# s-will/BiAlign

Hardware: AMD Instinct MI355X
Metric: giga-DP-cells/sec (higher is better)
Workload: dtype int32

## Files before the change

### bialign_amd/csrc/bialign_capi.hip

```cpp
#include "bialign_host.hpp"
#include <cmath>
#include <cstdint>
#include <unordered_map>

using namespace bialign;

namespace bialign {

static thread_local std::string g_err;

int fail(int code, const char* fmt, ...) {
  char buf[512];
  va_list ap;
  va_start(ap, fmt);
  vsnprintf(buf, sizeof buf, fmt, ap);
  va_end(ap);
  g_err = buf;
  return code;
}

struct SweepInfo {
  int W, R, RR, MAXOFF, PADB;
  int recdw, lean_recdw;
  int blk, min_goff;
// ... 434 lines not shown
  for (int t = 0; t < sc->k1 * sc->k1; ++t) amax = std::max<int64_t>(amax, std::llabs((long long)sc->s1[t]));
  int64_t bmax = 0;
  for (int t = 0; t < sc->k2 * sc->k2; ++t) bmax = std::max<int64_t>(bmax, std::llabs((long long)sc->s2[t]));
  auto dense_max = [&](const int32_t* tab, const int64_t* off) {
    int64_t mx = 0;
    for (int p = 0; p < pr->npairs; ++p) {
      const int64_t cnt = (int64_t)std::max(pr->len_a[p], 0) * std::max(pr->len_b[p], 0);
      for (int64_t t = 0; t < cnt; ++t) mx = std::max<int64_t>(mx, std::llabs((long long)tab[off[p] + t]));
    }
    return mx;
  };
  if (b->dense && !b->feat) bmax = dense_max(pr->mu2_dense, pr->mu2_off);
  if (b->feat) {
    struct MolMax { int32_t len; double up, down, unp; };
    std::unordered_map<int64_t, MolMax> seen[2];
    auto check = [&](int side, int p, int64_t off, int32_t len, const double* up, const double* down, const double* unp,
                     const MolMax** res) {
      MolMax& mm = seen[side][off];
      if (mm.len < len) {
        const double* arr[3] = {up, down, unp};
        static const char* const names[3] = {"up", "down", "unp"};
        double mx[3] = {0, 0, 0};
        for (int f = 0; f < 3; ++f)
          for (int32_t r = 0; r < len; ++r) {
            const double x = arr[f][off + r];
            if (!(x >= 0.0) || std::isinf(x))
              return fail(BIALIGN_E_INVALID, "pair %d: feature %s_%c at position %d is %g: features must be finite and >= 0", p,
                          names[f], side ? 'b' : 'a', r + 1, x);
            mx[f] = std::max(mx[f], x);
          }
        mm = MolMax{len, mx[0], mx[1], mx[2]};
      }
      *res = &mm;
      return BIALIGN_OK;
    };
    bmax = 0;
    for (int p = 0; p < pr->npairs; ++p) {
      const MolMax *ma = nullptr, *mb = nullptr;
      if (int rc = check(0, p, pr->off_a[p], std::max(pr->len_a[p], 0), ft->up_a, ft->down_a, ft->unp_a, &ma)) return rc;
      if (int rc = check(1, p, pr->off_b[p], std::max(pr->len_b[p], 0), ft->up_b, ft->down_b, ft->unp_b, &mb)) return rc;
      const double bound = std::fabs((double)ft->structure_weight) *
                           (std::sqrt(ma->up * mb->up) + std::sqrt(ma->down * mb->down) + std::sqrt(ma->unp * mb->unp));
      if (!(bound < 1073741824.0))
        return fail(BIALIGN_E_RANGE, "pair %d: structure scores may leave the int32 safety window (bound %g)", p, bound);
      bmax = std::max<int64_t>(bmax, (int64_t)std::ceil(bound));
    }
  }
  if (b->dense1) amax = dense_max(pr->mu1_dense, pr->mu1_off);
  const int64_t colmax = amax + bmax + 2 * (std::llabs((long long)prm->gap_cost) + std::llabs((long long)prm->gap_opening_cost)) +
                         2 * std::llabs((long long)prm->shift_cost);

  int64_t tot_a = 0, tot_b = 0, tot_tab = 0;
  b->pairs.resize(pr->npairs);
  std::vector<int64_t> pair_dwords(pr->npairs);
  for (int p = 0; p < pr->npairs; ++p) {
    const int n = pr->len_a[p], m = pr->len_b[p];
    if (n < 1 || m < 1)
      return fail(BIALIGN_E_INVALID, "pair %d: empty molecule (n=%d, m=%d)", p, n, m);
    if ((2 * ((int64_t)n + m) + 8) * colmax >= (1 << 28))
      return fail(BIALIGN_E_RANGE, "pair %d: scores may leave the int32 safety window (n+m=%d, column bound %lld)", p,
                  n + m, (long long)colmax);
    PairDesc& d = b->pairs[p];
    d.n = n;
    d.m = m;
    d.NS = d.P = d.G = 0;
    if (!b->wide) sweep_geometry(geo, n, m, &d.NS, &d.P, &d.G);
    d.trace_cap = 2 * (n + m) + 2;
    d.seq_a = pr->off_a[p];
    d.seq_b = pr->off_b[p];
    d.trace_off = b->trace_bytes;
    d.tab_off = tot_tab;
    tot_tab += (int64_t)n * m * ((b->dense ? 1 : 0) + (b->dense1 ? 1 : 0));
    if (b->feat) b->tab_dwords.push_back((int64_t)n * m * (b->dense1 ? 2 : 1));
    b->trace_bytes += d.trace_cap;
    b->cells += cells_of(n, m, S);
    tot_a = std::max<int64_t>(tot_a, pr->off_a[p] + n);
    tot_b = std::max<int64_t>(tot_b, pr->off_b[p] + m);
    if (!b->wide) {
      b->lds_bytes = std::max(b->lds_bytes, lds_need(geo, 1, sc->k1, sc->k2, n, m, b->dense, false, b->dense1));
      b->lds_base = std::max(b->lds_base, lds_need(geo, 0, sc->k1, sc->k2, n, m, b->dense, false, b->dense1));
      b->lds_diet8 = std::max(b->lds_diet8, lds_need(geo, 8, sc->k1, sc->k2, n, m, false, true));
      b->lds_slim_codes = std::max(b->lds_slim_codes, lds_need_slim_codes(geo, n, m));
    }
    b->lds_trace = std::max<size_t>(b->lds_trace, ((size_t)sc->k1 * sc->k1 + (size_t)sc->k2 * sc->k2) * 4 +
                                                      (b->dense1 ? 1 : 2) * ((size_t)code_pad(n) + (size_t)code_pad(m)));
  }
  if (!b->wide)
    b->lds_per_wave = lds_need(geo, 1, sc->k1, sc->k2, 1, 1, b->dense, false, b->dense1) -
                      lds_need(geo, 0, sc->k1, sc->k2, 1, 1, b->dense, false, b->dense1);
  if (!b->wide) b->lds_slim_base = lds_need_slim_base(geo, sc->k1, sc->k2);
  if (std::max(b->lds_bytes, b->lds_trace) > 160 * 1024)
    return fail(BIALIGN_E_UNSUPPORTED, "molecules too long for the LDS staging (%zu bytes needed, 160 KiB per workgroup)",
                std::max(b->lds_bytes, b->lds_trace));

  {
    const char* e = getenv("BIALIGN_PACK");
    const bool force = e && e[0] == '1';
    const PackInfo pki = pack_info(S);
    bool ok = b->affine && S >= 1 && S <= BIALIGN_MAX_SHIFT_PACKED && !b->lean && !b->dense1 && prm->gap_opening_cost <= 0 &&
              !(e && e[0] == '0') &&
              (force || colmax < 8192) &&
              (force || S < 3 || pr->npairs >= 64);
    for (int p = 0; ok && p < pr->npairs; ++p) {
      const PairDesc& d = b->pairs[p];
      const int interior = d.m - S - pki.lo + 1;
      const int64_t packed_dw = pki.written_dwords(d.G, d.P, d.m);
      const int64_t full_dw = (int64_t)d.G * pki.full_recdw;
      ok = interior >= 1 && (force || packed_dw * 5 <= full_dw * 4);
    }
    b->pack = ok;
  }

  size_t free_b = 0, total_b = 0;
  HIP_TRY(hipMemGetInfo(&free_b, &total_b));
  free_b += (eng->layer_cache.n + eng->layer_cache2.n) * sizeof(int32_t);
  if (b->feat) free_b += eng->tab_cache.n * sizeof(int32_t);
  int64_t budget = hbm_budget > 0 ? hbm_budget : (int64_t)(free_b * 0.85);
  budget = std::min<int64_t>(budget, (int64_t)(free_b * 0.95));
  const int64_t budget_dw = budget / 4;
  auto size_pairs = [&]() {
    for (int p = 0; p < pr->npairs; ++p) {
      PairDesc& d = b->pairs[p];
      if (b->wide) {
        pair_dwords[p] = b->lean ? 16 : wide_pair_dwords(d.n, d.m, S, b->NL);
        continue;
      }
      const int64_t lean_dw = (int64_t)d.G * geo.lean_recdw;
      const int64_t scratch_dw = (int64_t)(d.m + geo.MAXOFF + 1) * geo.recdw;
      d.scratch_off = lean_dw;
      pair_dwords[p] = b->lean_trace ? lean_dw + b->resw_k * scratch_dw : (b->lean ? lean_dw : (int64_t)d.G * geo.recdw);
      if (b->pack && !b->lean)
        pair_dwords[p] = pack_info(S).pair_dwords(d.G, d.P, d.m);
    }
  };
  auto max_need = [&]() {
    int64_t mx = 0;
    for (int p = 0; p < pr->npairs; ++p) mx = std::max(mx, pair_dwords[p] + (b->feat ? b->tab_dwords[p] : 0));
    return mx;
  };
  auto pick_resw_k = [&]() {
    int ns_max = 1;
    for (const PairDesc& d : b->pairs) ns_max = std::max(ns_max, d.NS);
    b->resw_k = (int)std::min<int64_t>(std::min<int64_t>(256, std::max(1, ns_max / 4)), std::max<int64_t>(1, 2048 / pr->npairs));
    if (const char* e = getenv("BIALIGN_RESW_K")) b->resw_k = std::min(256, std::max(1, atoi(e)));
    for (size_pairs(); b->resw_k > 1 && max_need() > budget_dw; size_pairs())
      b->resw_k /= 2;
  };
  if (b->lean_trace) pick_resw_k();
  size_pairs();
  if (b->pack) {
    int64_t full_max = 0;
    for (int p = 0; p < pr->npairs; ++p)
      full_max = std::max(full_max, (int64_t)b->pairs[p].G * pack_info(S).full_recdw + (b->feat ? b->tab_dwords[p] : 0));
    if (std::max(full_max, max_need()) > budget_dw) {
      b->pack = false;
      size_pairs();
    }
  }
  if (!b->lean && !b->wide && max_need() > budget_dw) {
    b->lean = b->lean_trace = true;
    b->pack = false;
    pick_resw_k();
  }
  b->full_dwords.resize(pr->npairs);
  for (int p = 0; p < pr->npairs; ++p) b->full_dwords[p] = b->wide ? pair_dwords[p] : (int64_t)b->pairs[p].G * geo.recdw;
  b->packed_sizing = b->pack && !b->lean;
  if (int rc = plan_chunks(b.get(), pair_dwords, budget_dw)) return rc;

// ... 438 lines not shown
```

### bialign_amd/csrc/bialign_host.hpp

```cpp
#pragma once
#include "bialign_kernels.hpp"

#include <algorithm>
#include <cstdarg>
#include <cstdio>
#include <cstdlib>
#include <cstring>
#include <memory>
#include <mutex>
#include <numeric>
#include <string>
#include <type_traits>
#include <vector>

#include "../../include/bialign.h"

#define BIALIGN_MAX_SHIFT_PACKED 3

namespace bialign {

int fail(int code, const char* fmt, ...);

#define HIP_TRY(expr)                                                                 \
  do {                                                                                \
// ... 313 lines not shown
  constexpr int PPW = 12 / TW;
  DeviceBatch w = v;
  w.order = v.order + first;
  w.team = 1;
  w.launch_pairs = count;
  w.slim_code_bytes = (int32_t)b->lds_slim_codes;
  b->packed_layers = !LEAN;
  if (!LEAN) b->used_pack = true;
  b->last_team = TW;
  return launch(fill_affine_slim_kernel<S, TW, PPW, LEAN>, dim3((count + PPW - 1) / PPW), dim3(64 * 12), b->lds_slim(TW),
                b->eng->stream, w);
}

template <int S, bool LEAN>
int launch_fill_affine_slim(bialign_batch* b, const DeviceBatch& v, int first, int count, int tw) {
  switch (tw) {
    case 2: return launch_fill_affine_slim_t<S, 2, LEAN>(b, v, first, count);
    case 3: return launch_fill_affine_slim_t<S, 3, LEAN>(b, v, first, count);
    case 6: return launch_fill_affine_slim_t<S, 6, LEAN>(b, v, first, count);
    case 12: return launch_fill_affine_slim_t<S, 12, LEAN>(b, v, first, count);
  }
  return fail(BIALIGN_E_UNSUPPORTED, "no three-waves-per-SIMD sweep for max_shift %d, team %d", S, tw);
}

template <int S, int TW, unsigned F>
int xcu_resident_affine(bialign_batch* b) {
  constexpr unsigned Q = (F & ~F_PACK) | F_XCU;
  if constexpr (fill_affine_exists(S, TW, Q)) {
    if (TW == 8 && !diet8_available(b)) return 0;
    return xcu_resident_cached(b, ((F & F_LEAN) ? 1 : 0) + (TW == 8 ? 2 : 0), fill_affine_of<S, TW, Q>(), 64 * TW, fill_lds<S, TW>(b, true));
  } else {
    return 0;
  }
}

template <int S, int TW, unsigned F>
bool fill_affine_rung(bialign_batch* b, const DeviceBatch& v, int first, int count, const TeamShape& ts, int* rc) {
  if constexpr (fill_affine_exists(S, TW, F)) {
    constexpr bool XCU = (F & F_XCU) != 0;
    if (XCU ? !(ts.gw > 1 && (TW == 1 || ts.tw == TW)) : ts.tw < TW) return false;
    *rc = launch_fill_affine_t<S, TW, F>(b, v, first, count, XCU ? ts.gw : 1);
    return true;
  } else {
    return false;
  }
}

template <int S>
int launch_fill_affine(bialign_batch* b, const DeviceBatch& v, int first, int count) {
  return with_flags<F_DENSE | F_LEAN | F_PACK | F_DENSE1 | F_BETA_ANY>(fill_flags(b), [&](auto flags) -> int {
    constexpr unsigned F = decltype(flags)::value;
    if constexpr (!fill_affine_exists(S, 1, F)) {
      return fail(BIALIGN_E_UNSUPPORTED, "no affine sweep for max_shift %d in form %u", S, F);
    } else {
      TeamShape ts;
      if constexpr (!(F & F_BETA_ANY)) ts = team_shape(b, first, count, xcu_resident_affine<S, 1, F>(b), xcu_resident_affine<S, 8, F>(b));
      if constexpr (fill_slim_exists(S, F)) {
        if (ts.slim) return launch_fill_affine_slim<S, (F & F_LEAN) != 0>(b, v, first, count, ts.tw);
      }
      int rc = BIALIGN_OK;
      (void)(fill_affine_rung<S, 8, F | F_XCU>(b, v, first, count, ts, &rc) || fill_affine_rung<S, 1, F | F_XCU>(b, v, first, count, ts, &rc) ||
             fill_affine_rung<S, 8, F>(b, v, first, count, ts, &rc) || fill_affine_rung<S, 4, F>(b, v, first, count, ts, &rc) ||
             fill_affine_rung<S, 2, F>(b, v, first, count, ts, &rc) || fill_affine_rung<S, 1, F>(b, v, first, count, ts, &rc));
      return rc;
    }
  });
}

template <int S>
int launch_resweep_affine(bialign_batch* b, const DeviceBatch& v, int first, int count) {
  DeviceBatch w = v;
  w.order = v.order + first;
  w.team = 1;
  return with_flags<F_DENSE | F_DENSE1 | F_BETA_ANY>(fill_flags(b), [&](auto flags) -> int {
    return launch(fill_affine_of<S, 1, decltype(flags)::value | F_RESW>(), dim3(count * b->resw_k), dim3(64), fill_lds<S, 1>(b, true),
                  b->eng->stream, w);
  });
}

inline unsigned trace_flags(const bialign_batch* b, bool do_trace) {
  return (do_trace ? T_TRACE : 0u) | (b->dense1 && do_trace ? T_DENSE1 : 0u) | (b->packed_layers ? T_PACK : 0u);
}
template <typename... P>
int launch_traceback_kernel(const bialign_batch* b, void (*kern)(P...), bool do_trace, const DeviceBatch& v, int first, int count) {
  DeviceBatch w = v;
  w.order = v.order + first;
  return launch(kern, dim3(count), dim3(64), do_trace ? b->lds_trace : 0, b->eng->stream, w, count);
}

template <int S>
int launch_traceback_affine(const bialign_batch* b, const DeviceBatch& v, int first, int count, bool do_trace) {
  return with_flags<T_TRACE | T_PACK | T_DENSE1>(trace_flags(b, do_trace), [&](auto flags) -> int {
    constexpr unsigned F = decltype(flags)::value;
    if constexpr (traceback_exists(true, S, F)) return launch_traceback_kernel(b, traceback_affine_of<S, F>(), do_trace, v, first, count);
    else return fail(BIALIGN_E_UNSUPPORTED, "no affine traceback for max_shift %d in form %u", S, F);
  });
}
template <int S>
int launch_traceback_affine_strip(const bialign_batch* b, const DeviceBatch& v, int first, int count) {
  return b->dense1 ? launch_traceback_kernel(b, traceback_affine_of<S, T_TRACE | T_STRIP | T_DENSE1>(), true, v, first, count)
                   : launch_traceback_kernel(b, traceback_affine_of<S, T_TRACE | T_STRIP>(), true, v, first, count);
}

template <int S, int TW, unsigned F>
int launch_fill_linear_t(bialign_batch* b, const DeviceBatch& v, int first, int count, int gw) {
  constexpr bool XCU = (F & F_XCU) != 0;
  DeviceBatch w = v;
  w.order = v.order + first;
  w.team = gw;
  b->packed_layers = false;
  b->last_team = XCU ? -gw : TW;
  const dim3 grid(count * (XCU ? gw : 1)), block(64 * TW);
  if (XCU) return launch_team(b, fill_linear_of<S, TW, F>(), grid, block, fill_lds<S, TW>(b, false), w, count, true);
  return launch(fill_linear_of<S, TW, F>(), grid, block, fill_lds<S, TW>(b, false), b->eng->stream, w);
}

template <int S, int TW, unsigned F>
bool fill_linear_rung(bialign_batch* b, const DeviceBatch& v, int first, int count, const TeamShape& ts, int* rc) {
  if constexpr (fill_linear_exists(TW, F)) {
    constexpr bool XCU = (F & F_XCU) != 0;
    if (XCU ? ts.gw <= 1 : ts.tw < TW) return false;
    *rc = launch_fill_linear_t<S, TW, F>(b, v, first, count, XCU ? ts.gw : 1);
    return true;
  } else {
    return false;
  }
}

template <int S>
int launch_fill_linear(bialign_batch* b, const DeviceBatch& v, int first, int count) {
  return with_flags<F_DENSE | F_LEAN | F_DENSE1>(fill_flags(b), [&](auto flags) -> int {
    constexpr unsigned F = decltype(flags)::value;
    const int resident = xcu_resident_cached(b, (F & F_LEAN) ? 1 : 0, fill_linear_of<S, 1, F | F_XCU>(), 64, fill_lds<S, 1>(b, false));
    const TeamShape ts = team_shape(b, first, count, resident);
    int rc = BIALIGN_OK;
    (void)(fill_linear_rung<S, 1, F | F_XCU>(b, v, first, count, ts, &rc) || fill_linear_rung<S, 8, F>(b, v, first, count, ts, &rc) ||
           fill_linear_rung<S, 4, F>(b, v, first, count, ts, &rc) || fill_linear_rung<S, 2, F>(b, v, first, count, ts, &rc) ||
           fill_linear_rung<S, 1, F>(b, v, first, count, ts, &rc));
    return rc;
  });
}

template <int S>
int launch_resweep_linear(bialign_batch* b, const DeviceBatch& v, int first, int count) {
  DeviceBatch w = v;
  w.order = v.order + first;
  return with_flags<F_DENSE | F_DENSE1>(fill_flags(b), [&](auto flags) -> int {
    return launch(fill_linear_of<S, 1, decltype(flags)::value | F_RESW>(), dim3(count * b->resw_k), dim3(64), fill_lds<S, 1>(b, false),
                  b->eng->stream, w);
  });
}

template <int S>
int launch_traceback_linear(const bialign_batch* b, const DeviceBatch& v, int first, int count, bool do_trace) {
  return with_flags<T_TRACE | T_DENSE1>(trace_flags(b, do_trace), [&](auto flags) -> int {
    constexpr unsigned F = decltype(flags)::value;
    if constexpr (traceback_exists(false, S, F)) return launch_traceback_kernel(b, traceback_linear_of<S, F>(), do_trace, v, first, count);
    else return fail(BIALIGN_E_UNSUPPORTED, "no one-layer traceback for max_shift %d in form %u", S, F);
  });
}
template <int S>
int launch_traceback_linear_strip(const bialign_batch* b, const DeviceBatch& v, int first, int count) {
  return b->dense1 ? launch_traceback_kernel(b, traceback_linear_of<S, T_TRACE | T_STRIP | T_DENSE1>(), true, v, first, count)
                   : launch_traceback_kernel(b, traceback_linear_of<S, T_TRACE | T_STRIP>(), true, v, first, count);
}

template <int S, int NL>
int launch_dump(const bialign_batch* b, const DeviceBatch& v, int pid, int32_t* d_out) {
  if constexpr (S >= 1 && S <= BIALIGN_MAX_SHIFT_PACKED && NL == 9) {
    if (b->packed_layers) return launch(dump_layers_kernel<S, NL, true>, dim3(256), dim3(256), 0, b->eng->stream, v, pid, d_out);
  }
  return launch(dump_layers_kernel<S, NL>, dim3(256), dim3(256), 0, b->eng->stream, v, pid, d_out);
}

int launch_fill_wide(bialign_batch* b, const DeviceBatch& v, int first, int count);
int launch_traceback_wide(const bialign_batch* b, const DeviceBatch& v, int first, int count, bool do_trace);
int launch_dump_wide(const bialign_batch* b, const DeviceBatch& v, int pid, int32_t* d_out);

#define BIALIGN_INST_KIND0(S, X)                                                                \
  X template int launch_fill_affine<S>(bialign_batch*, const DeviceBatch&, int, int);          \
  X template int launch_resweep_affine<S>(bialign_batch*, const DeviceBatch&, int, int);
#define BIALIGN_INST_KIND1(S, X)                                                                         \
  X template int launch_fill_linear<S>(bialign_batch*, const DeviceBatch&, int, int);                   \
  X template int launch_traceback_affine<S>(const bialign_batch*, const DeviceBatch&, int, int, bool);  \
  X template int launch_traceback_affine_strip<S>(const bialign_batch*, const DeviceBatch&, int, int);  \
  X template int launch_traceback_linear<S>(const bialign_batch*, const DeviceBatch&, int, int, bool);  \
  X template int launch_resweep_linear<S>(bialign_batch*, const DeviceBatch&, int, int);                \
  X template int launch_traceback_linear_strip<S>(const bialign_batch*, const DeviceBatch&, int, int);  \
  X template int launch_dump<S, 9>(const bialign_batch*, const DeviceBatch&, int, int32_t*);            \
  X template int launch_dump<S, 1>(const bialign_batch*, const DeviceBatch&, int, int32_t*);
#define BIALIGN_FOR_EACH_S(M, X) M(0, X) M(1, X) M(2, X) M(3, X) M(4, X) M(5, X)

#ifndef BIALIGN_TU_S
BIALIGN_FOR_EACH_S(BIALIGN_INST_KIND0, extern)
BIALIGN_FOR_EACH_S(BIALIGN_INST_KIND1, extern)
#endif

}
```

### bialign_amd/csrc/bialign_traceback.hpp

```cpp
#pragma once

namespace bialign {

__device__ __forceinline__ int shift_of(int hU, int hV) {
  return hU == hV ? 0 : ((hU == 2 || hV == 2) ? 1 : 2);
}

struct TraceInputs {
  const int32_t *s1, *s2;
  const uint8_t *sa, *ca, *sb, *cb;
};
template <bool D1 = false>
__device__ __forceinline__ TraceInputs stage_trace_inputs(const DeviceBatch& A, const PairDesc& pd,
                                                          int32_t* smem) {
  const int k1 = A.k1, k2 = A.k2, n = pd.n, m = pd.m;
  int32_t* s1 = smem;
  int32_t* s2 = s1 + k1 * k1;
  uint8_t* sa = reinterpret_cast<uint8_t*>(s2 + k2 * k2);
  uint8_t* ca = sa + (D1 ? 0 : code_pad(n));
  uint8_t* sb = ca + code_pad(n);
  uint8_t* cb = sb + (D1 ? 0 : code_pad(m));
  for (int t = threadIdx.x; t < k1 * k1; t += 64) s1[t] = A.s1[t];
  for (int t = threadIdx.x; t < k2 * k2; t += 64) s2[t] = A.s2[t];
  for (int t = threadIdx.x; t < n; t += 64) {
    if (!D1) sa[t] = A.seq_a[pd.seq_a + t];
    ca[t] = A.cls_a[pd.seq_a + t];
  }
  for (int t = threadIdx.x; t < m; t += 64) {
    if (!D1) sb[t] = A.seq_b[pd.seq_b + t];
    cb[t] = A.cls_b[pd.seq_b + t];
  }
  __syncthreads();
  return TraceInputs{s1, s2, sa, ca, sb, cb};
}

__device__ __forceinline__ int wave_min16(int v) {
  v = min(v, __builtin_amdgcn_update_dpp(v, v, 0x128 , 0xf, 0xf, false));
  v = min(v, __builtin_amdgcn_update_dpp(v, v, 0x124 , 0xf, 0xf, false));
  v = min(v, __builtin_amdgcn_update_dpp(v, v, 0x122 , 0xf, 0xf, false));
  v = min(v, __builtin_amdgcn_update_dpp(v, v, 0x121 , 0xf, 0xf, false));
  return v;
}

template <int S, bool DO_TRACE, bool STRIP = false, bool WIDE = false, bool PACK = false, bool D1 = false>
__global__ void __launch_bounds__(64) traceback_affine_kernel(const DeviceBatch A, int npairs) {
  static_assert(!WIDE || !STRIP, "no lean traceback on the wide-band path");
  static_assert(!PACK || (!WIDE && !STRIP), "packed records: full-storage tiled sweeps");
  const int SR = WIDE ? A.wide_s : S;
  const int pid = A.order[blockIdx.x];
  const PairDesc pd = A.pairs[pid];
  const int n = pd.n, m = pd.m;
  const int beta = A.beta, gamma = A.gamma, delta = A.delta;
  const int32_t* lay = A.layers;
  const int c = threadIdx.x;
  constexpr int BIG = 0x7fffffff;
  constexpr int W = 2 * S + 1, RR = Geo<S>::RR;
  extern __shared__ __align__(16) int32_t smem[];

  TraceState ts{};
  if (STRIP) {
    ts = A.tstate[pid];
    if (ts.done) return;
  }
  const int Q = STRIP ? (ts.started ? ts.strip : pd.NS - 1) : 0;
  const int Qlo = STRIP ? max(Q - A.resw_k + 1, 0) : 0;
  const int64_t sstride = (int64_t)(m + Geo<S>::MAXOFF + 1) * Rec<S, 9>::RECDW;
  auto cell = [&](int pi, int pj, int a, int b, int ss) -> int {
    if (WIDE) return lay[pd.layer_off + wide_dword(m, 2 * SR + 1, 9, pi, pj, a, b, ss)];
    if (PACK) return packed_cell<S>(lay, pd, pi, pj, a, b, ss);
    if (!STRIP) return lay[cell_dword<S, 9>(pd, pi, pj, a, b, ss)];
    const int sp = pi / RR, ilp = pi - sp * RR + 1;
    if (sp >= Qlo)
      return A.scratch[pd.scratch_off + (Q - sp) * sstride +
                       Rec<S, 9>::dword(pj + 2 * ilp + a, (ilp - 1) * W + a, b * 9 + ss)];
    return lay[pd.layer_off + Rec<S, 9, true>::dword((int64_t)sp * pd.P + pj + 2 * ilp + a, a, b * 9 + ss)];
  };

  int i = n, j = m, k = n, l = m, d0 = 0, d1 = 0, len = 0, complete = 0;
  int st = 0, cur = 0;
  if (!STRIP || !ts.started) {
    const int endv = c < 9 ? cell(n, m, SR, SR, c) : -BIG;
    const int best = __builtin_amdgcn_readfirstlane(-wave_min16(-endv));
    if (c == 0) A.scores[pid] = best;
    if (!DO_TRACE) return;
    const int skey = (c < 9 && endv == best) ? (shift_of(c / 3, c % 3) << 4 | c) : BIG;
    st = __builtin_amdgcn_readfirstlane(wave_min16(skey)) & 15;
    cur = best;
  } else {
    i = ts.i; j = ts.j; k = ts.k; l = ts.l; st = ts.st; cur = ts.cur; d0 = ts.d0; d1 = ts.d1; len = ts.len;
  }
  const TraceInputs in = stage_trace_inputs<D1>(A, pd, smem);
  const uint8_t *sa = in.sa, *ca = in.ca, *sb = in.sb, *cb = in.cb;
  const int32_t* const mu1tab = D1 ? mu1_table(A, pd) : nullptr;

  uint8_t* out = A.trace + pd.trace_off;
  bool finished = true;
  const int grp = c < 9 ? 1 : (c < 12 ? 2 : 3);
  const int hfree = grp == 2 ? 2 - (c - 9) : 2 - (c - 12);
  while (true) {
    if (i == 0 && j == 0 && k == 0 && l == 0 && st == 8) { complete = 1; break; }
    if (STRIP && i < Qlo * RR) { finished = false; break; }
    const int hU = st / 3, hV = st - 3 * hU;
    const int u0 = hU >= 1, u1 = hU != 1, v0 = hV >= 1, v1 = hV != 1;
    const int mu1 = (i >= 1 && j >= 1)
                        ? (D1 ? mu1tab[(int64_t)(i - 1) * m + (j - 1)] : in.s1[sa[i - 1] * A.k1 + sb[j - 1]])
                        : 0;
    const int mu2 = (k >= 1 && l >= 1)
                        ? ((D1 ? (A.dense_forms & 1) != 0 : A.dense_tab != nullptr)
                               ? A.dense_tab[pd.tab_off + (int64_t)(k - 1) * m + (l - 1)]
                               : in.s2[ca[k - 1] * A.k2 + cb[l - 1]])
                        : 0;
    const int valU = hU == 2 ? mu1 : gamma, valV = hV == 2 ? mu2 : gamma;

    const int o0 = grp == 2 ? 0 : u0, o1 = grp == 2 ? 0 : u1;
    const int o2 = grp == 3 ? 0 : v0, o3 = grp == 3 ? 0 : v1;
    const int ss = grp == 1 ? c : (grp == 2 ? 3 * hU + hfree : 3 * hfree + hV);
    const int ra = ss / 3, rb = ss - 3 * ra;
    const int openU = (hU != 2 && ra != hU) ? beta : 0, openV = (hV != 2 && rb != hV) ? beta : 0;
    const int sc = grp == 1   ? delta * shift_of(hU, hV) + valU + valV + openU + openV
                   : grp == 2 ? delta * (v0 + v1) + valV + openV
                              : delta * (u0 + u1) + valU + openU;
    const int pi = i - o0, pj = j - o1, pk = k - o2, pl = l - o3;
    const bool ok = c < 15 && pi >= 0 && pj >= 0 && pk >= 0 && pl >= 0 && abs(pk - pi) <= SR &&
                    abs(pl - pj) <= SR;
    const int ld = ok ? cell(pi, pj, pk - pi + SR, pl - pj + SR, ss) : 0;
    const int r0 = ra >= 1, r1 = ra != 1, r2 = rb >= 1, r3 = rb != 1;
    const int t0 = d0 + (o0 - o2) + (r0 - r2), t1 = d1 + (o1 - o3) + (r1 - r3);
    const int key = (ok && ld + sc == cur) ? ((abs(t0) + abs(t1)) << 16 | abs(t1) << 8 | c) : BIG;
    const int kmin = __builtin_amdgcn_readfirstlane(wave_min16(key));
    if (kmin == BIG) break;
    const int pick = kmin & 63;
    const int code = __builtin_amdgcn_readlane(o0 * 8 + o1 * 4 + o2 * 2 + o3, pick);
    st = __builtin_amdgcn_readlane(ss, pick);
    cur = __builtin_amdgcn_readlane(ld, pick);
    const int q0 = (code >> 3) & 1, q1 = (code >> 2) & 1, q2 = (code >> 1) & 1, q3 = code & 1;
    d0 += q0 - q2;
    d1 += q1 - q3;
    if (c == 0 && len < pd.trace_cap) out[len] = (uint8_t)code;
    ++len;
    i -= q0; j -= q1; k -= q2; l -= q3;
  }
  if (STRIP && !finished) {
    if (c == 0) {
      TraceState nx;
      nx.i = i; nx.j = j; nx.k = k; nx.l = l; nx.st = st; nx.cur = cur; nx.d0 = d0; nx.d1 = d1;
      nx.len = len; nx.strip = Qlo - 1; nx.started = 1; nx.done = 0;
      A.tstate[pid] = nx;
    }
    return;
  }
  if (len > pd.trace_cap) len = pd.trace_cap;
  __builtin_amdgcn_s_waitcnt(0);
  __syncthreads();
  for (int x = c; x < len / 2; x += 64) {
    const uint8_t t = out[x];
    out[x] = out[len - 1 - x];
    out[len - 1 - x] = t;
  }
  if (c == 0) {
    A.trace_len[pid] = len;
    A.complete[pid] = complete;
    if (STRIP) {
      ts.done = 1;
      ts.started = 1;
      A.tstate[pid] = ts;
    }
  }
}

template <int S, bool DO_TRACE, bool STRIP = false, bool WIDE = false, bool D1 = false>
__global__ void __launch_bounds__(64) traceback_linear_kernel(const DeviceBatch A, int npairs) {
  static_assert(!WIDE || !STRIP, "no lean traceback on the wide-band path");
  const int SR = WIDE ? A.wide_s : S;
  const int pid = A.order[blockIdx.x];
  const PairDesc pd = A.pairs[pid];
  const int n = pd.n, m = pd.m;
  const int gamma = A.gamma, delta = A.delta;
  const int32_t* lay = A.layers;
  const int c = threadIdx.x;
  constexpr int BIG = 0x7fffffff;
  constexpr int W = 2 * S + 1, RR = Geo<S>::RR;
  extern __shared__ __align__(16) int32_t smem[];
  TraceState ts{};
  if (STRIP) {
    ts = A.tstate[pid];
    if (ts.done) return;
  }
  const int Q = STRIP ? (ts.started ? ts.strip : pd.NS - 1) : 0;
  const int Qlo = STRIP ? max(Q - A.resw_k + 1, 0) : 0;
  const int64_t sstride = (int64_t)(m + Geo<S>::MAXOFF + 1) * Rec<S, 1>::RECDW;
  auto cell = [&](int pi, int pj, int a, int b) -> int {
    if (WIDE) return lay[pd.layer_off + wide_dword(m, 2 * SR + 1, 1, pi, pj, a, b, 0)];
    if (!STRIP) return lay[cell_dword<S, 1>(pd, pi, pj, a, b, 0)];
    const int sp = pi / RR, ilp = pi - sp * RR + 1;
    if (sp >= Qlo)
      return A.scratch[pd.scratch_off + (Q - sp) * sstride + Rec<S, 1>::dword(pj + 2 * ilp + a, (ilp - 1) * W + a, b)];
    return lay[pd.layer_off + Rec<S, 1, true>::dword((int64_t)sp * pd.P + pj + 2 * ilp + a, a, b)];
  };
  int cur = (STRIP && ts.started) ? ts.cur : cell(n, m, SR, SR);
  if (c == 0 && !(STRIP && ts.started)) A.scores[pid] = cur;
  if (!DO_TRACE) return;
  const TraceInputs in = stage_trace_inputs<D1>(A, pd, smem);
  const uint8_t *sa = in.sa, *ca = in.ca, *sb = in.sb, *cb = in.cb;
  const int32_t* const mu1tab = D1 ? mu1_table(A, pd) : nullptr;

  constexpr int OFF[16] = {15, 10, 5, 12, 3, 8, 4, 2, 1, 11, 7, 14, 13, 0, 0, 0};
  int code_c = 0;
#pragma unroll
  for (int t = 0; t < 13; ++t)
    if (c == t) code_c = OFF[t];
  const int o0 = (code_c >> 3) & 1, o1 = (code_c >> 2) & 1, o2 = (code_c >> 1) & 1, o3 = code_c & 1;
  const int use1 = (c == 0 || c == 3 || c == 11 || c == 12), use2 = (c == 0 || c == 4 || c == 9 || c == 10);
  const int gD = gamma + delta;
  const int kconst = c == 0 ? 0 : (c <= 2 ? 2 * gamma : (c <= 4 ? delta : gD));

  uint8_t* out = A.trace + pd.trace_off;
  int i = n, j = m, k = n, l = m, len = 0;
  if (STRIP && ts.started) { i = ts.i; j = ts.j; k = ts.k; l = ts.l; len = ts.len; }
  bool finished = true;
  while (true) {
    if (STRIP && i < Qlo * RR) { finished = false; break; }
    const int mu1 = (i >= 1 && j >= 1)
                        ? (D1 ? mu1tab[(int64_t)(i - 1) * m + (j - 1)] : in.s1[sa[i - 1] * A.k1 + sb[j - 1]])
                        : 0;
    const int mu2 = (k >= 1 && l >= 1)
                        ? ((D1 ? (A.dense_forms & 1) != 0 : A.dense_tab != nullptr)
                               ? A.dense_tab[pd.tab_off + (int64_t)(k - 1) * m + (l - 1)]
                               : in.s2[ca[k - 1] * A.k2 + cb[l - 1]])
                        : 0;
    const int sc = kconst + (use1 ? mu1 : 0) + (use2 ? mu2 : 0);
    const int pi = i - o0, pj = j - o1, pk = k - o2, pl = l - o3;
    const bool ok = c < 13 && pi >= 0 && pj >= 0 && pk >= 0 && pl >= 0 && abs(pk - pi) <= SR && abs(pl - pj) <= SR;
    const int ld = ok ? cell(pi, pj, pk - pi + SR, pl - pj + SR) : 0;
    const int key = (ok && ld + sc == cur) ? c : BIG;
    const int pick = __builtin_amdgcn_readfirstlane(wave_min16(key));
    if (pick == BIG) break;
    const int code = __builtin_amdgcn_readlane(code_c, pick);
    cur = __builtin_amdgcn_readlane(ld, pick);
    if (c == 0 && len < pd.trace_cap) out[len] = (uint8_t)code;
    ++len;
    i -= (code >> 3) & 1; j -= (code >> 2) & 1; k -= (code >> 1) & 1; l -= code & 1;
  }
  if (STRIP && !finished) {
    if (c == 0) {
      TraceState nx{};
      nx.i = i; nx.j = j; nx.k = k; nx.l = l; nx.cur = cur; nx.len = len;
      nx.strip = Qlo - 1; nx.started = 1; nx.done = 0;
      A.tstate[pid] = nx;
    }
    return;
  }
  if (len > pd.trace_cap) len = pd.trace_cap;
  __builtin_amdgcn_s_waitcnt(0);
  __syncthreads();
  for (int x = c; x < len / 2; x += 64) {
    const uint8_t t = out[x];
    out[x] = out[len - 1 - x];
    out[len - 1 - x] = t;
  }
  if (c == 0) {
    A.trace_len[pid] = len;
    A.complete[pid] = 1;
    if (STRIP) {
      ts.done = 1;
      ts.started = 1;
      A.tstate[pid] = ts;
    }
  }
}

}
```

### bialign_amd/csrc/bialign_types.hpp

```cpp
#pragma once

namespace bialign {

constexpr int32_t NEG = -(1 << 30);
constexpr int32_t SENT = -(1 << 30) - (1 << 29);
constexpr int32_t THRESH = -(1 << 30) - (1 << 28);
constexpr int NCOL = 65;
constexpr int PROG_WORDS = 256;
constexpr int LDS_PROG_WORDS = 16;
constexpr int XCH_ROWS = 12;
__host__ __device__ constexpr int code_pad(int len, int guard = 0) { return (len + 2 * guard + 3) & ~3; }
typedef int v4i __attribute__((ext_vector_type(4)));

struct PairDesc {
  int32_t n, m;
  int32_t NS, P, G;
  int32_t trace_cap;
  int64_t seq_a, seq_b;
  int64_t layer_off;
  int64_t trace_off;
  int64_t tab_off;
  int64_t scratch_off;
};

// ... 72 lines not shown
  return (bb == 0 && (st == 3 || st == 5 || st == 6)) || (bb == W - 1 && (st == 1 || st == 2 || st == 7));
}

template <int S>
struct Pack {
  using G_ = Geo<S>;
  using R_ = Rec<S, 9>;
  static constexpr int ND = R_::ND;
  static constexpr int ANCHOR = 8;
  static constexpr int NHW = ND + 1;
  static constexpr int NDW = (NHW + 1) / 2;
  static constexpr int NCH = NDW / 4 + (NDW % 4 == 3 ? 1 : 0);
  static constexpr int TAILDW = NDW % 4 == 3 ? 0 : NDW % 4;
  static constexpr int NPC = NCH + (TAILDW ? 1 : 0);
  static constexpr int TSLOTS = TAILDW == 0 ? 0 : (TAILDW == 2 ? (R_::SL + 1) / 2 * 2 : (R_::SL + 3) / 4 * 4);
  static constexpr int RECDW = NCH * R_::CH + TSLOTS * TAILDW;
  static_assert(RECDW % 4 == 0, "packed records must stay 16-byte aligned");
  __host__ __device__ static constexpr int hw(int v) { return 2 + v - (v > ANCHOR ? 1 : 0); }
  __host__ __device__ static constexpr int val(int h) { return h - 2 < ANCHOR ? h - 2 : h - 1; }
  __host__ __device__ static constexpr int dwpos(int slot, int d) {
    return d < 4 * NCH ? (d >> 2) * R_::CH + slot * 4 + (d & 3) : NCH * R_::CH + slot * TAILDW + (d - 4 * NCH);
  }
  static constexpr int LO = S + 1 + G_::MAXOFF;
  static constexpr int Q0 = (S + 2 + G_::RR - 1) / G_::RR;
  __host__ __device__ static inline int hi(int m) { return m - S; }
  __host__ __device__ static inline bool interior(int qs, int c, int m) { return qs >= Q0 && c >= LO && c <= m - S; }
  __host__ __device__ static inline int nbs(int P, int m) { return P - (m - S - LO + 1); }
  __host__ __device__ static inline int64_t bidx(int qs, int c, int P, int m) {
    if (qs < Q0) return (int64_t)qs * P + c;
    return (int64_t)Q0 * P + (int64_t)(qs - Q0) * nbs(P, m) + (c < LO ? c : c - (m - S + 1) + LO);
  }
  __host__ __device__ static inline int64_t full_records(int G, int P, int m) {
    const int nst = (G + P - 1) / P;
    return nst <= Q0 ? (int64_t)nst * P : (int64_t)Q0 * P + (int64_t)(nst - Q0) * nbs(P, m);
  }
  __host__ __device__ static inline int64_t pair_dwords(int G, int P, int m) {
    return (int64_t)G * RECDW + full_records(G, P, m) * R_::RECDW;
  }
  __host__ __device__ static inline int64_t written_dwords(int G, int P, int m) {
    const int64_t f = full_records(G, P, m);
    return (G - f) * RECDW + f * R_::RECDW;
  }
  __host__ __device__ static inline uint32_t offset_of(uint32_t h, int base) { return (h - (uint32_t)base) & 0xffffu; }
  typedef unsigned short pk_u16x2 __attribute__((ext_vector_type(2)));
  __device__ static inline uint32_t offsets_of(uint32_t word, int base) {
    const pk_u16x2 w = __builtin_bit_cast(pk_u16x2, word);
    const unsigned short b = (unsigned short)base;
    return __builtin_bit_cast(uint32_t, (pk_u16x2)(w - pk_u16x2{b, b}));
  }
  __host__ __device__ static inline int decode(const int32_t* p, int slot, int bb, int st, bool corner) {
    const int v = bb * 9 + st;
    const int base = p[slot * 4];
    if (v == ANCHOR) return base + 0x8000;
    const int h = hw(v);
    const uint32_t word = (uint32_t)p[dwpos(slot, h >> 1)];
    const uint32_t e = offset_of((h & 1) ? word >> 16 : word & 0xffffu, base);
    return (corner && e == 0xffffu) ? NEG : base + (int)e;
  }
};

template <int S>
__host__ __device__ inline int packed_cell(const int32_t* layers, const PairDesc& pd, int i, int j, int aa, int bb, int st) {
  using PK = Pack<S>;
  constexpr int W = 2 * S + 1, RR = Geo<S>::RR;
  const int strip = i / RR, il = i - strip * RR + 1;
  const int t = j + 2 * il + aa, over = t >= pd.P ? 1 : 0;
  const int slot = (il - 1) * W + aa;
  const int32_t* base = layers + pd.layer_off;
  if (PK::interior(strip + over, t - over * pd.P, pd.m))
    return PK::decode(base + ((int64_t)strip * pd.P + t) * PK::RECDW, slot, bb, st, pack_corner(W, st, bb));
  return base[(int64_t)pd.G * PK::RECDW + PK::bidx(strip + over, t - over * pd.P, pd.P, pd.m) * Rec<S, 9>::RECDW +
              Rec<S, 9>::dword(0, slot, bb * 9 + st)];
}

template <int S, int NL>
__host__ __device__ inline int64_t cell_dword(const PairDesc& pd, int i, int j, int aa, int bb,
                                              int st) {
  constexpr int W = 2 * S + 1, RR = Geo<S>::RR;
  const int strip = i / RR, il = i - strip * RR + 1;
  const int64_t g = (int64_t)strip * pd.P + j + 2 * il + aa;
  return pd.layer_off + Rec<S, NL>::dword(g, (il - 1) * W + aa, bb * NL + st);
}

}
```

Measured before the change: 205.7.

## Stage traceback cell records into an LDS window tile

Traceback kernels now prefetch a (K+1)x(K+1) tile of DP records around the current cell into LDS with coalesced, unrolled vector loads, and decode packed records during the fill. Cell lookups read from that window, which is refilled whenever the path leaves it. This targets the serial, latency-bound global loads of the single-wave traceback walk, at the cost of extra LDS per workgroup and some records loaded that the path never visits. The window size is chosen on the host under an LDS budget and can be overridden by an environment variable.

```diff
diff --git a/bialign_amd/csrc/bialign_capi.hip b/bialign_amd/csrc/bialign_capi.hip
--- a/bialign_amd/csrc/bialign_capi.hip
+++ b/bialign_amd/csrc/bialign_capi.hip
@@ -540,8 +540,7 @@
       b->lds_diet8 = std::max(b->lds_diet8, lds_need(geo, 8, sc->k1, sc->k2, n, m, false, true));
       b->lds_slim_codes = std::max(b->lds_slim_codes, lds_need_slim_codes(geo, n, m));
     }
-    b->lds_trace = std::max<size_t>(b->lds_trace, ((size_t)sc->k1 * sc->k1 + (size_t)sc->k2 * sc->k2) * 4 +
-                                                      (b->dense1 ? 1 : 2) * ((size_t)code_pad(n) + (size_t)code_pad(m)));
+    b->lds_trace = std::max<size_t>(b->lds_trace, trace_inputs_bytes(sc->k1, sc->k2, n, m, b->dense1));
   }
   if (!b->wide)
     b->lds_per_wave = lds_need(geo, 1, sc->k1, sc->k2, 1, 1, b->dense, false, b->dense1) -
diff --git a/bialign_amd/csrc/bialign_host.hpp b/bialign_amd/csrc/bialign_host.hpp
--- a/bialign_amd/csrc/bialign_host.hpp
+++ b/bialign_amd/csrc/bialign_host.hpp
@@ -419,17 +419,35 @@
   return (do_trace ? T_TRACE : 0u) | (b->dense1 && do_trace ? T_DENSE1 : 0u) | (b->packed_layers ? T_PACK : 0u);
 }
 template <typename... P>
-int launch_traceback_kernel(const bialign_batch* b, void (*kern)(P...), bool do_trace, const DeviceBatch& v, int first, int count) {
+int launch_traceback_kernel(const bialign_batch* b, void (*kern)(P...), bool do_trace, const DeviceBatch& v, int first, int count,
+                            int win_k = 0, size_t win_bytes = 0) {
   DeviceBatch w = v;
   w.order = v.order + first;
-  return launch(kern, dim3(count), dim3(64), do_trace ? b->lds_trace : 0, b->eng->stream, w, count);
+  return launch(kern, dim3(count), dim3(64), do_trace ? b->lds_trace + win_bytes : 0, b->eng->stream, w, count, do_trace ? win_k : 0);
+}
+
+constexpr int TRACE_WINDOW_KMAX = 8;
+template <int S, int NL>
+int trace_window_k(const bialign_batch* b) {
+  using TW = TraceWin<S, NL, false>;
+  if (const char* e = getenv("BIALIGN_TRACE_WINDOW")) {
+    int k = std::max(0, std::min(atoi(e), 64));
+    while (k > 0 && b->lds_trace + TW::bytes(k) > 160 * 1024) --k;
+    return k;
+  }
+  int k = TRACE_WINDOW_KMAX;
+  while (k > 0 && (b->lds_trace + TW::bytes(k) > 40 * 1024 || TW::records(k) > 64 * TW::UNROLL)) --k;
+  return k >= 2 ? k : 0;
 }
 
 template <int S>
 int launch_traceback_affine(const bialign_batch* b, const DeviceBatch& v, int first, int count, bool do_trace) {
   return with_flags<T_TRACE | T_PACK | T_DENSE1>(trace_flags(b, do_trace), [&](auto flags) -> int {
     constexpr unsigned F = decltype(flags)::value;
-    if constexpr (traceback_exists(true, S, F)) return launch_traceback_kernel(b, traceback_affine_of<S, F>(), do_trace, v, first, count);
+    if constexpr (traceback_exists(true, S, F)) {
+      const int k = trace_window_k<S, 9>(b);
+      return launch_traceback_kernel(b, traceback_affine_of<S, F>(), do_trace, v, first, count, k, TraceWin<S, 9, false>::bytes(k));
+    }
     else return fail(BIALIGN_E_UNSUPPORTED, "no affine traceback for max_shift %d in form %u", S, F);
   });
 }
@@ -492,7 +510,10 @@
 int launch_traceback_linear(const bialign_batch* b, const DeviceBatch& v, int first, int count, bool do_trace) {
   return with_flags<T_TRACE | T_DENSE1>(trace_flags(b, do_trace), [&](auto flags) -> int {
     constexpr unsigned F = decltype(flags)::value;
-    if constexpr (traceback_exists(false, S, F)) return launch_traceback_kernel(b, traceback_linear_of<S, F>(), do_trace, v, first, count);
+    if constexpr (traceback_exists(false, S, F)) {
+      const int k = trace_window_k<S, 1>(b);
+      return launch_traceback_kernel(b, traceback_linear_of<S, F>(), do_trace, v, first, count, k, TraceWin<S, 1, false>::bytes(k));
+    }
     else return fail(BIALIGN_E_UNSUPPORTED, "no one-layer traceback for max_shift %d in form %u", S, F);
   });
 }
diff --git a/bialign_amd/csrc/bialign_traceback.hpp b/bialign_amd/csrc/bialign_traceback.hpp
--- a/bialign_amd/csrc/bialign_traceback.hpp
+++ b/bialign_amd/csrc/bialign_traceback.hpp
@@ -42,8 +42,74 @@
   return v;
 }
 
+template <int S, int NL, bool PACK>
+__device__ __forceinline__ void trace_window_fill(const int32_t* lay, const PairDesc& pd, int32_t* win, int K, int wi0,
+                                                  int wj0) {
+  using TW = TraceWin<S, NL, PACK>;
+  using R_ = Rec<S, NL>;
+  constexpr int W = TW::W, ND = TW::ND, U = TW::UNROLL, NCH4 = R_::NCH4, TAIL = R_::TAIL;
+  constexpr int PNCH = PACK ? Pack<PACK ? S : 1>::NCH : 0, PTAIL = PACK ? Pack<PACK ? S : 1>::TAILDW : 0;
+  constexpr int NT = TAIL > PTAIL ? TAIL : PTAIL;
+  const int side = K + 1, nrec = side * side * W;
+  for (int r0 = 0; r0 < nrec; r0 += 64 * U) {
+    v4i ch[U][NCH4 > 0 ? NCH4 : 1];
+    int tl[U][NT > 0 ? NT : 1];
+    bool live[U], pk[U];
+    int wbase[U];
+#pragma unroll
+    for (int u = 0; u < U; ++u) {
+      const int r = r0 + u * 64 + (int)threadIdx.x;
+      const int q = r / W, a = r - q * W, di = q / side, dj = q - di * side;
+      const int pi = wi0 + di, pj = wj0 + dj;
+      live[u] = r < nrec && pi >= 0 && pj >= 0;
+      const typename TW::Src s = live[u] ? TW::source(pd, pi, pj, a) : TW::source(pd, wi0 + K, wj0 + K, 0);
+      pk[u] = s.packed;
+      wbase[u] = r * ND;
+      const int64_t first = pd.layer_off;
+#pragma unroll
+      for (int k = 0; k < NCH4; ++k) {
+        const int64_t at = (k == 0 || !s.packed || k < PNCH) ? TW::raw_dword(s, 4 * k) : first;
+        ch[u][k] = *reinterpret_cast<const v4i*>(lay + at);
+      }
+#pragma unroll
+      for (int t = 0; t < NT; ++t) {
+        const int64_t at = s.packed ? (t < PTAIL ? TW::raw_dword(s, 4 * PNCH + t) : first)
+                                    : (t < TAIL ? TW::raw_dword(s, 4 * NCH4 + t) : first);
+        tl[u][t] = lay[at];
+      }
+    }
+    auto raw = [&](int u, int d, int nch) -> int {
+      const int k = d >> 2, t = d - 4 * nch;
+      return d < 4 * nch ? ch[u][k < NCH4 ? k : 0][d & 3] : tl[u][t >= 0 && t < NT ? t : 0];
+    };
+#pragma unroll
+    for (int u = 0; u < U; ++u) {
+      if (!live[u]) continue;
+      int32_t* const dst = win + wbase[u];
+#pragma unroll
+      for (int v = 0; v < ND; ++v) {
+        int val = raw(u, v, NCH4);
+        if constexpr (PACK) {
+          using PK = Pack<S>;
+          const int base = ch[u][0][0];
+          int pv = base + 0x8000;
+          if (v != PK::ANCHOR) {
+            const int h = PK::hw(v);
+            const uint32_t word = (uint32_t)raw(u, h >> 1, PNCH);
+            const uint32_t e = PK::offset_of((h & 1) ? word >> 16 : word & 0xffffu, base);
+            pv = (pack_corner(W, v % 9, v / 9) && e == 0xffffu) ? NEG : base + (int)e;
+          }
+          val = pk[u] ? pv : val;
+        }
+        dst[v] = val;
+      }
+    }
+  }
+  __syncthreads();
+}
+
 template <int S, bool DO_TRACE, bool STRIP = false, bool WIDE = false, bool PACK = false, bool D1 = false>
-__global__ void __launch_bounds__(64) traceback_affine_kernel(const DeviceBatch A, int npairs) {
+__global__ void __launch_bounds__(64) traceback_affine_kernel(const DeviceBatch A, int npairs, int K) {
   static_assert(!WIDE || !STRIP, "no lean traceback on the wide-band path");
   static_assert(!PACK || (!WIDE && !STRIP), "packed records: full-storage tiled sweeps");
   const int SR = WIDE ? A.wide_s : S;
@@ -65,7 +131,22 @@
   const int Q = STRIP ? (ts.started ? ts.strip : pd.NS - 1) : 0;
   const int Qlo = STRIP ? max(Q - A.resw_k + 1, 0) : 0;
   const int64_t sstride = (int64_t)(m + Geo<S>::MAXOFF + 1) * Rec<S, 9>::RECDW;
+  constexpr bool WIN = DO_TRACE && !STRIP && !WIDE;
+  using TWin = TraceWin<S, 9, PACK && WIN>;
+  int32_t* win = nullptr;
+  int wi0 = 0, wj0 = 0;
+  if constexpr (WIN) {
+    if (K > 0) {
+      win = smem + trace_inputs_bytes(A.k1, A.k2, n, m, D1) / 4;
+      wi0 = n - K;
+      wj0 = m - K;
+      trace_window_fill<S, 9, PACK && WIN>(lay, pd, win, K, wi0, wj0);
+    }
+  }
   auto cell = [&](int pi, int pj, int a, int b, int ss) -> int {
+    if constexpr (WIN) {
+      if (K > 0) return win[TWin::slot(K, pi - wi0, pj - wj0, a, b, ss)];
+    }
     if (WIDE) return lay[pd.layer_off + wide_dword(m, 2 * SR + 1, 9, pi, pj, a, b, ss)];
     if (PACK) return packed_cell<S>(lay, pd, pi, pj, a, b, ss);
     if (!STRIP) return lay[cell_dword<S, 9>(pd, pi, pj, a, b, ss)];
@@ -100,6 +181,13 @@
   while (true) {
     if (i == 0 && j == 0 && k == 0 && l == 0 && st == 8) { complete = 1; break; }
     if (STRIP && i < Qlo * RR) { finished = false; break; }
+    if constexpr (WIN) {
+      if (K > 0 && ((i > 0 && i - 1 < wi0) || (j > 0 && j - 1 < wj0))) {
+        wi0 = i - K;
+        wj0 = j - K;
+        trace_window_fill<S, 9, PACK && WIN>(lay, pd, win, K, wi0, wj0);
+      }
+    }
     const int hU = st / 3, hV = st - 3 * hU;
     const int u0 = hU >= 1, u1 = hU != 1, v0 = hV >= 1, v1 = hV != 1;
     const int mu1 = (i >= 1 && j >= 1)
@@ -169,7 +257,7 @@
 }
 
 template <int S, bool DO_TRACE, bool STRIP = false, bool WIDE = false, bool D1 = false>
-__global__ void __launch_bounds__(64) traceback_linear_kernel(const DeviceBatch A, int npairs) {
+__global__ void __launch_bounds__(64) traceback_linear_kernel(const DeviceBatch A, int npairs, int K) {
   static_assert(!WIDE || !STRIP, "no lean traceback on the wide-band path");
   const int SR = WIDE ? A.wide_s : S;
   const int pid = A.order[blockIdx.x];
@@ -189,7 +277,22 @@
   const int Q = STRIP ? (ts.started ? ts.strip : pd.NS - 1) : 0;
   const int Qlo = STRIP ? max(Q - A.resw_k + 1, 0) : 0;
   const int64_t sstride = (int64_t)(m + Geo<S>::MAXOFF + 1) * Rec<S, 1>::RECDW;
+  constexpr bool WIN = DO_TRACE && !STRIP && !WIDE;
+  using TWin = TraceWin<S, 1, false>;
+  int32_t* win = nullptr;
+  int wi0 = 0, wj0 = 0;
+  if constexpr (WIN) {
+    if (K > 0) {
+      win = smem + trace_inputs_bytes(A.k1, A.k2, n, m, D1) / 4;
+      wi0 = n - K;
+      wj0 = m - K;
+      trace_window_fill<S, 1, false>(lay, pd, win, K, wi0, wj0);
+    }
+  }
   auto cell = [&](int pi, int pj, int a, int b) -> int {
+    if constexpr (WIN) {
+      if (K > 0) return win[TWin::slot(K, pi - wi0, pj - wj0, a, b, 0)];
+    }
     if (WIDE) return lay[pd.layer_off + wide_dword(m, 2 * SR + 1, 1, pi, pj, a, b, 0)];
     if (!STRIP) return lay[cell_dword<S, 1>(pd, pi, pj, a, b, 0)];
     const int sp = pi / RR, ilp = pi - sp * RR + 1;
@@ -220,6 +323,13 @@
   bool finished = true;
   while (true) {
     if (STRIP && i < Qlo * RR) { finished = false; break; }
+    if constexpr (WIN) {
+      if (K > 0 && ((i > 0 && i - 1 < wi0) || (j > 0 && j - 1 < wj0))) {
+        wi0 = i - K;
+        wj0 = j - K;
+        trace_window_fill<S, 1, false>(lay, pd, win, K, wi0, wj0);
+      }
+    }
     const int mu1 = (i >= 1 && j >= 1)
                         ? (D1 ? mu1tab[(int64_t)(i - 1) * m + (j - 1)] : in.s1[sa[i - 1] * A.k1 + sb[j - 1]])
                         : 0;
diff --git a/bialign_amd/csrc/bialign_types.hpp b/bialign_amd/csrc/bialign_types.hpp
--- a/bialign_amd/csrc/bialign_types.hpp
+++ b/bialign_amd/csrc/bialign_types.hpp
@@ -178,4 +178,45 @@
   return pd.layer_off + Rec<S, NL>::dword(g, (il - 1) * W + aa, bb * NL + st);
 }
 
-}
+__host__ __device__ constexpr size_t trace_inputs_bytes(int k1, int k2, int n, int m, bool dense1) {
+  return ((size_t)k1 * k1 + (size_t)k2 * k2) * 4 + (dense1 ? 1 : 2) * ((size_t)code_pad(n) + (size_t)code_pad(m));
+}
+
+template <int S, int NL, bool PACK>
+struct TraceWin {
+  using R_ = Rec<S, NL>;
+  static constexpr int W = 2 * S + 1, ND = NL * W, RR = Geo<S>::RR;
+  static constexpr int UNROLL = 128 / ND < 1 ? 1 : (128 / ND > 4 ? 4 : 128 / ND);
+  __host__ __device__ static constexpr int records(int K) { return (K + 1) * (K + 1) * W; }
+  __host__ __device__ static constexpr size_t bytes(int K) { return K > 0 ? (size_t)records(K) * ND * 4 : 0; }
+  __host__ __device__ static constexpr int slot(int K, int di, int dj, int a, int b, int st) {
+    return ((di * (K + 1) + dj) * W + a) * ND + b * NL + st;
+  }
+  struct Src {
+    int64_t rec;
+    int slot;
+    bool packed;
+  };
+  __host__ __device__ static inline Src source(const PairDesc& pd, int pi, int pj, int a) {
+    const int strip = pi / RR, il = pi - strip * RR + 1;
+    const int t = pj + 2 * il + a, slot = (il - 1) * W + a;
+    if constexpr (PACK) {
+      using PK = Pack<S>;
+      const int over = t >= pd.P ? 1 : 0;
+      if (PK::interior(strip + over, t - over * pd.P, pd.m))
+        return Src{pd.layer_off + ((int64_t)strip * pd.P + t) * PK::RECDW, slot, true};
+      return Src{pd.layer_off + (int64_t)pd.G * PK::RECDW + PK::bidx(strip + over, t - over * pd.P, pd.P, pd.m) * R_::RECDW,
+                 slot, false};
+    } else {
+      return Src{pd.layer_off + ((int64_t)strip * pd.P + t) * R_::RECDW, slot, false};
+    }
+  }
+  __host__ __device__ static inline int64_t raw_dword(const Src& s, int d) {
+    if constexpr (PACK) {
+      if (s.packed) return s.rec + Pack<S>::dwpos(s.slot, d);
+    }
+    return s.rec + R_::dword(0, s.slot, d);
+  }
+};
+
+}
```

New measurement: 206.7 (median of 6 runs). About the same (+0.5%).
